# wgrosche/AIrcraft

Hardware: AMD Instinct MI355X
Metric: MPC horizon-steps/sec (6-DoF+NN-surrogate RK4, step + A,B sensitivities) at H=50, batch=4096 (higher is better)
Workload: dtype f32

## Files before the change

### aircraft_amd/build.py

```python
from __future__ import annotations

import glob
import os
import subprocess
import sys
from concurrent.futures import ThreadPoolExecutor

_HERE = os.path.dirname(os.path.abspath(__file__))
CSRC = os.path.join(_HERE, "csrc")
OBJ = os.path.join(_HERE, "csrc", "_obj")
OUT = os.path.join(_HERE, "libaircraft_hip.so")
HEADERS = glob.glob(os.path.join(CSRC, "*.hpp")) + [os.path.join(_HERE, "..", "include", "aircraft_hip.h")]
CFLAGS = ["--offload-arch=gfx950", "-O3", "-std=c++17", "-fPIC", "-fno-gpu-rdc", "-Wno-pass-failed", "-ffp-contract=on"]
UNIT_FLAGS = {
    "an_inst_sens_poly": ["-fno-slp-vectorize"],
    "nn_inst_wt2_mfma_sens_w2": ["-fno-slp-vectorize"],
    "nn_inst_wt8_mfma_sens": ["-DAC_CH=2", "-mllvm", "-slp-threshold=6", "-mllvm", "-amdgpu-mfma-vgpr-form"],
    "nn_inst_wt8_mfma_pair": ["-DAC_CH=2", "-mllvm", "-slp-threshold=6", "-mllvm", "-amdgpu-mfma-vgpr-form"],
    "nn_inst_wt8_f16_sens": ["-DAC_CH=2", "-mllvm", "-slp-threshold=6", "-mllvm", "-amdgpu-mfma-vgpr-form"],
    "nn_inst_wt8_f16_pair": ["-DAC_CH=2", "-mllvm", "-slp-threshold=6", "-mllvm", "-amdgpu-mfma-vgpr-form"],
}


def sources():
    return sorted(glob.glob(os.path.join(CSRC, "*.hip")))


def source_sha() -> str:
    import hashlib

    hh = hashlib.sha256()
    for f in sources() + sorted(HEADERS):
        hh.update(os.path.basename(f).encode())
        with open(f, "rb") as fh:
            hh.update(fh.read())
    hh.update(repr((CFLAGS, sorted(UNIT_FLAGS.items()))).encode())
    return hh.hexdigest()[:16]


def _deps(obj):
    d = obj + ".d"
    if not os.path.exists(d):
        return HEADERS
# ... 50 lines not shown
```

### aircraft_amd/csrc/ac_mlp.hpp

```cpp
#pragma once
#include "ac_dynamics.hpp"
#include "ac_mlp_plan.hpp"

namespace ac {

typedef float f32x4 __attribute__((ext_vector_type(4)));

#ifdef AC_HIDDEN_FP32
constexpr bool kBf16Hidden = false;
#else
constexpr bool kBf16Hidden = true;
#endif
constexpr int kHiddenFp32 = 0, kHiddenBf16 = 1, kHiddenF16 = 2;
constexpr int kDefaultHidden = kBf16Hidden ? kHiddenBf16 : kHiddenFp32;

__device__ __attribute__((noinline)) inline f32x4 mma_16x16x4_valu(float a, float b, f32x4 c) {
    const int lane = threadIdx.x & 63, col = lane & 15, g = lane >> 4;
#pragma unroll
    for (int k = 0; k < 4; ++k) {
        const float bk = __shfl(b, col + 16 * k, 64);
#pragma unroll
        for (int r = 0; r < 4; ++r) c[r] = fmaf(__shfl(a, 4 * g + r + 16 * k, 64), bk, c[r]);
    }
    return c;
}

template <bool USE_MFMA> AC_DI f32x4 mma_16x16x4(float a, float b, f32x4 c) {
    if constexpr (USE_MFMA) return __builtin_amdgcn_mfma_f32_16x16x4f32(a, b, c, 0, 0, 0);
    else return mma_16x16x4_valu(a, b, c);
}

AC_DI float act_tanh(float x) {
    const float e = __builtin_amdgcn_exp2f(x * 2.8853900817779268f);
    return 1.0f - 2.0f * __builtin_amdgcn_rcpf(1.0f + e);
}

// ... 11 lines not shown

template <bool ON> struct TripleHolder {
    int tri_p = 0, tri_q = 1, tri_r = 2, tri_t = 3;
    AC_DI void set_triple(int p, int q, int r) { tri_p = p; tri_q = q; tri_r = r; }
    AC_DI void set_quad(int p, int q, int r, int t) { tri_p = p; tri_q = q; tri_r = r; tri_t = t; }
    AC_DI int tri(int i) const { return i == 0 ? tri_p : i == 1 ? tri_q : i == 2 ? tri_r : tri_t; }
};
template <> struct TripleHolder<false> {
    AC_DI int tri(int) const { return 0; }
};

template <bool ON> struct BfRingState {
    int bf_front = 0;
    const char* bf_back = nullptr;
    const float* bf_next_src = nullptr;
    int bf_next_dst = 0;
};
template <> struct BfRingState<false> {};

template <int NSLAB, int WT, bool USE_MFMA, bool TANGENT = (NSLAB == 6), bool SECOND = false, int TOFF = 0, int PAIR = 0,
          int HID = kHiddenFp32>
struct MlpEngine : TripleHolder<SECOND && NSLAB <= 10>, BfRingState<HID != kHiddenFp32> {
    static constexpr bool BF = HID != kHiddenFp32;
    static constexpr bool F16 = HID == kHiddenF16;
    static constexpr int NP = F16 ? 2 : 3;
    static constexpr int NPROD = F16 ? 3 : 6;
    using TripleHolder<SECOND && NSLAB <= 10>::tri;
    static constexpr bool kNoValue = PAIR == 2;
    static constexpr int kFirstTangent = kNoValue ? 0 : 1;
    static_assert(PAIR == 0 || (TANGENT && USE_MFMA && NSLAB == 3), "wave-pair roles: three slabs each, matrix-core flavour");
    static_assert(!BF || (TANGENT && USE_MFMA && WT == 8), "bf16 hidden layers: the width-128 sensitivity engines");
    static_assert(!TANGENT || (NSLAB >= 2 && NSLAB <= 6 && TOFF + NSLAB - kFirstTangent <= 5), "tangent mode = value + a range of the 5 input tangents");
    static constexpr int kTangents = TANGENT ? NSLAB - kFirstTangent : 0;
    static_assert(!SECOND || ((NSLAB == 9 || NSLAB == 10 || NSLAB == 21) && !TANGENT), "second-order mode: 9 (bipartite), 10 (triple) or 21 (all five inputs) slabs");
    static constexpr int kFirstOrder = !SECOND ? 0 : (NSLAB == 10 ? 3 : NSLAB == 9 ? 4 : 5);
    AC_DI static constexpr int second_a(int s) {
        constexpr int K = kFirstOrder;
        if (NSLAB == 9) return s < 7 ? 1 : 2;
        if (s <= 2 * K) return s - K;
        int m = s - 2 * K - 1;
        for (int i = 1; i < K; ++i) { if (m < K - i) return i; m -= K - i; }
        return K;
    }
    AC_DI static constexpr int second_b(int s) {
        constexpr int K = kFirstOrder;
        if (NSLAB == 9) return (s & 1) ? 3 : 4;
        if (s <= 2 * K) return s - K;
// ... 23 lines not shown
    static constexpr bool kSpread = TANGENT && NSLAB * (WT / CH) * 4 >= WT * WT + 1;
    const char* dma_src;
    unsigned dma_dst;
    int dma_last;

    AC_DI MlpEngine(const MlpPlan& pl, const float* blob, char* lds_base)
        : plan(pl), gblob(blob), lds(lds_base), ring_pos(0), snext(pl.n_streamed > 1 ? 1 : 0),
          dma_src((const char*)(blob + pl.g_off[0])), dma_dst((unsigned)pl.lds_off[0]), dma_last(0) {
        lane = threadIdx.x & 63; g = lane >> 4; wave = threadIdx.x >> 6; nwaves = blockDim.x >> 6;
    }

    AC_DI int streamed_layer(int idx) const {
        int seen = 0;
        for (int l = 0; l < plan.n_layers; ++l)
            if (plan.lds_off[l] < 0) { if (seen == idx) return l; ++seen; }
        return -1;
    }

    AC_DI void load_weights() {
        for (int l = 0; l < plan.n_layers; ++l)
            if (plan.lds_off[l] >= 0) lds_dma_copy(gblob + plan.g_off[l], lds + plan.lds_off[l], plan.bytes[l], wave, nwaves, lane);
        if constexpr (BF) {
            if (!kPairRing && plan.n_streamed > 0)
                lds_dma_copy(gblob + plan.g_off[plan.first_streamed], lds + plan.bf_region[0], kBfFront, wave, nwaves, lane);
        } else if (plan.n_streamed > 0) {
            const int l = plan.first_streamed;
            lds_dma_copy(gblob + plan.g_off[l], lds + plan.ring_off[0], plan.bytes[l], wave, nwaves, lane);
        }
        asm volatile("s_waitcnt vmcnt(0)" ::: "memory");
        __syncthreads();
    }

    AC_DI void drain() { asm volatile("s_waitcnt vmcnt(0)" ::: "memory"); }

    template <int NT, int ACT = -1>
    AC_DI void epilogue_tile(int s, int nt, const f32x4 (&o)[NT], int act_flag) {
        const bool act = ACT < 0 ? act_flag != 0 : ACT != 0;
#pragma unroll
        for (int r = 0; r < 4; ++r) {
            if constexpr (kNoValue) {
                a[s][nt][r] = o[nt][r];
            } else if (s == 0 || !kDeriv) {
                a[s][nt][r] = act ? act_tanh(o[nt][r]) : o[nt][r];
            } else if (!SECOND || s <= kFirstOrder) {
                const float h = a[0][nt][r];
                a[s][nt][r] = act ? o[nt][r] * fmaf(-h, h, 1.0f) : o[nt][r];
            } else {
// ... 130 lines not shown
                const bool more = !(s == NSLAB - 1 && nc + C >= NT);
                gemm_chunk<C, KT, NT, ACT>(wf, bias4, s, nc, o[s & 1], a[s], o[(s + 1) & 1], act, wcur, bcur, more);
            }
            if (KT == WT && NT == WT) { if (s == 0) AC_MARK(st, 9); else if (s == 1) AC_MARK(st, 10); else AC_MARK(st, 11); }
            if constexpr (PAIR != 0 && KT == WT && NT == WT) {
                if (s == 1) {
                    __syncthreads();
                    if constexpr (PAIR == 1) {
#pragma unroll
                        for (int nt = 0; nt < WT; ++nt) hx[nt * 64 + lane] = f32x4{a[0][nt][0], a[0][nt][1], a[0][nt][2], a[0][nt][3]};
                    }
                }
            }
        }
#pragma unroll
        for (int nt = 0; nt < NT; ++nt) epilogue_tile<NT, ACT>(NSLAB - 1, nt, o[(NSLAB - 1) & 1], act);
    }

    typedef __bf16 bf16x8 __attribute__((ext_vector_type(8)));
    typedef unsigned u32x4 __attribute__((ext_vector_type(4)));
    static constexpr int KC = WT / 2;
    static constexpr bool kPairRing = PAIR != 0;
    static constexpr int kBfFront = (WT / 2) * KC * NP * 1024 + 1024, kBfBack = (WT / 2) * KC * NP * 1024;

    typedef float f32x2 __attribute__((ext_vector_type(2)));
    AC_DI static unsigned cvt_pk_bf16(f32x2 xy) {
        typedef __bf16 bf16x2 __attribute__((ext_vector_type(2)));
        return __builtin_bit_cast(unsigned, __builtin_convertvector(xy, bf16x2));
    }
    AC_DI static unsigned cvt_pk_bf16(float x, float y) { return cvt_pk_bf16(f32x2{x, y}); }
    typedef _Float16 f16x8 __attribute__((ext_vector_type(8)));
    template <bool H, class A, class B> struct PickFrag { typedef A type; };
    template <class A, class B> struct PickFrag<true, A, B> { typedef B type; };
    typedef typename PickFrag<F16, bf16x8, f16x8>::type frag8;
    static constexpr float kLoScale = 2048.0f, kLoInv = 1.0f / 2048.0f;
    AC_DI static unsigned cvt_pk_f16(f32x2 xy) {
        typedef _Float16 f16x2 __attribute__((ext_vector_type(2)));
        return __builtin_bit_cast(unsigned, __builtin_convertvector(xy, f16x2));
    }
    AC_DI static float sub_f16_lo(float x, unsigned u) {
        float d;
        asm volatile("v_fma_mix_f32 %0, %1, -1.0, %2 op_sel_hi:[1,0,0]" : "=v"(d) : "v"(u), "v"(x));
        return d;
    }
    AC_DI static float sub_f16_hi(float x, unsigned u) {
        float d;
// ... 2 lines not shown
    }
    AC_DI static unsigned scale_f16_lo(float r) {
        unsigned q;
        asm volatile("v_fma_mixlo_f16 %0, %1, %2, 0" : "=v"(q) : "v"(r), "s"(kLoScale));
        return q;
    }
    AC_DI static unsigned scale_f16_hi(unsigned q, float r) {
        asm volatile("v_fma_mixhi_f16 %0, %1, %2, 0" : "+v"(q) : "v"(r), "s"(kLoScale));
        return q;
    }
    AC_DI static f32x4 mfma_bf(const frag8& w, const frag8& x, f32x4 c) {
        if constexpr (F16) return __builtin_amdgcn_mfma_f32_16x16x32_f16(w, x, c, 0, 0, 0);
        else return __builtin_amdgcn_mfma_f32_16x16x32_bf16(w, x, c, 0, 0, 0);
    }
    AC_DI static float bf_sum(float hi, float lo) {
        if constexpr (F16) return fmaf(lo, kLoInv, hi);
        else return hi + lo;
    }
    AC_DI static frag8 ds_frag(unsigned lds_addr, int off) {
        frag8 v;
        asm volatile("ds_read_b128 %0, %1 offset:%2" : "=a"(v) : "v"(lds_addr), "i"(off));
        return v;
    }
    AC_DI static void wait_frags() {
        asm volatile("s_waitcnt lgkmcnt(0)" ::: "memory");
        __builtin_amdgcn_sched_barrier(0);
    }
    AC_DI void mid_layer() {
#ifdef AC_STAMPS_MID
        AC_MARK(st, 9);
        asm volatile("s_waitcnt vmcnt(0)" ::: "memory");
        AC_MARK(st, 6);
        __syncthreads();
        AC_MARK(st, 0);
#else
        asm volatile("s_waitcnt vmcnt(0)" ::: "memory");
        __syncthreads();
#endif
        if constexpr (!kPairRing) lds_dma_copy(this->bf_next_src, lds + this->bf_next_dst, kBfFront, wave, nwaves, lane);
    }

    static constexpr int NG = WT / CH;
    static constexpr int kTail = 2;
    static constexpr int kHead = (NG - kTail) * KC;
    static constexpr int NB = NG * KC;
    static constexpr int NGAP = NPROD * CH;
// ... 47 lines not shown
    static constexpr int NU = 2 * WT + 4 * KC;
    AC_DI static constexpr int unit_slab(int S, int B, int u) {
        if (u < WT) {
            const int sb = sum_blk(u / CH);
            return sb % NB == B ? (sb < NB ? S : S - 1) : -1;
        }
        if (u < 2 * WT) {
            const int t = u - WT;
            if (!kNoValue) {
                const int tb = tanh_blk(t);
                if ((S == 0 && tb == B) || (S == 1 && tb == NB + B)) return 0;
            }
            if (S >= kFirstTangent && epi_own(S, t) && epi_own_blk(t) == B) return S;
            if (S > kFirstTangent && !epi_own(S - 1, t) && epi_blk(S - 1, t) == B) return S - 1;
            return -1;
        }
        const int pb = split_blk((u - 2 * WT) / 4, (u - 2 * WT) % 4);
        if (pb < NB) return (pb == B && S + 1 < NSLAB) ? S + 1 : -1;
        return (pb == NB + B && S > 0) ? S : -1;
    }
    AC_DI static constexpr int unit_stages(int us, int u) {
        return u < WT ? 2 : u < 2 * WT ? (!kNoValue && us == 0 ? 12 : 4) : (F16 ? 3 : 6);
    }
    AC_DI static constexpr int gap_share(int S, int B) {
        if (!F16) return 1;
        int t = 0;
        for (int u = 0; u < NU; ++u) {
            const int us = unit_slab(S, B, u);
            if (us >= 0) t += unit_stages(us, u);
        }
        const int per = (t + NGAP - 1) / NGAP;
        return per < 1 ? 1 : per;
    }
    static constexpr int kSumGap = F16 ? NGAP / 2 : 4;
    AC_DI static constexpr int gap_stage(int S, int B, int J, int n) {
        const int per = gap_share(S, B);
        int j = 0;
        for (int v = WT; v < NU + WT; ++v) {
            const int u = v % NU;
            const int us = unit_slab(S, B, u);
            if (us < 0) continue;
            if (u < WT && j < kSumGap * per) j = kSumGap * per;
            for (int k = 0; k < unit_stages(us, u); ++k, ++j)
                if ((j / per < NGAP ? j / per : NGAP - 1) == J && n-- == 0) return u * 16 + k;
        }
        return -1;
    }

    struct BfRegs {
        f32x4 o[2][WT], hi[2][WT], lo[2][WT];
        u32x4 xq[WT / 2][NP];
        frag8 w[2][CH][NP];
        unsigned la0, la1;
        const f32x4* bias4;
        f32x2 sxy[2 * WT]; float tt[WT][4];
        unsigned su[2 * WT], sa[2 * WT], sb[2 * WT];
    };
    AC_DI static void bf_pin(float& v) { asm volatile("" : "+v"(v)); }
    AC_DI static void bf_pin(unsigned& v) { asm volatile("" : "+v"(v)); }

    template <int S, int B, int U, int K> AC_DI void bf_stage(BfRegs& r) {
        constexpr int us = unit_slab(S, B, U);
        constexpr bool early = S == 0 && B < kHead;
        if constexpr (U < WT) {
#pragma unroll
            for (int e = 2 * K; e < 2 * K + 2; ++e) {
                float v = bf_sum(r.hi[us & 1][U][e], r.lo[us & 1][U][e]);
                bf_pin(v);
                r.o[us & 1][U][e] = v;
// ... 60 lines not shown

    AC_DI frag8 bf_frag(const BfRegs& r, int nt, int c, int p) const {
        return ds_frag(nt < WT / 2 ? r.la0 : r.la1, (((nt % (WT / 2)) * KC + c) * NP + p) * 1024);
    }
    template <int S, int B, int J, int N> AC_DI void bf_gap_stages(BfRegs& r) {
        constexpr int e = gap_stage(S, B, J, N);
        if constexpr (e >= 0) {
            bf_stage<S, B, e / 16, e % 16>(r);
            bf_gap_stages<S, B, J, N + 1>(r);
        }
    }

    template <int S, int B, int J> AC_DI void bf_gap(BfRegs& r) {
        constexpr int nc = blk_group(B) * CH, c = blk_chunk(B), cur = B & 1, i = J % CH, m = J / CH;
        constexpr bool more = !(S + 1 == NSLAB && B + 1 == NB);
        constexpr int nb = (B + 1) % NB, nnc = blk_group(nb) * CH, nkc = blk_chunk(nb);
        constexpr int wp = F16 ? (m == 0 ? 1 : 0) : m == 0 ? 2 : (m == 1 || m == 4 || m == 5) ? 0 : 1;
        constexpr int xp = F16 ? (m == 1 ? 1 : 0) : m == 1 ? 2 : (m == 2 || m == 4) ? 1 : 0;
        const frag8 x = __builtin_bit_cast(frag8, r.xq[c][xp]);
        if constexpr (m < NPROD - 1) r.lo[S & 1][nc + i] = mfma_bf(r.w[cur][i][wp], x, r.lo[S & 1][nc + i]);
        else r.hi[S & 1][nc + i] = mfma_bf(r.w[cur][i][wp], x, r.hi[S & 1][nc + i]);
        __builtin_amdgcn_sched_barrier(0);
        if constexpr (more && J < NP * CH) r.w[cur ^ 1][J / NP][J % NP] = bf_frag(r, nnc + J / NP, nkc, J % NP);
        static_assert(F16 || gap_stage(S, B, J, 2) < 0, "at most two stages to a gap");
        bf_gap_stages<S, B, J, 0>(r);
        __builtin_amdgcn_sched_barrier(0);
        if constexpr (J + 1 < NGAP) bf_gap<S, B, J + 1>(r);
    }

    template <int S, int B> AC_DI void bf_block(BfRegs& r) {
        constexpr int nc = blk_group(B) * CH, c = blk_chunk(B);
        constexpr int nnc = blk_group((B + 1) % NB) * CH;
        __builtin_amdgcn_sched_barrier(0);
        if constexpr (S == 0 && nc < WT / 2 && nnc >= WT / 2) { mid_layer(); __builtin_amdgcn_sched_barrier(0); }
        wait_frags();
        if constexpr (c == 0) {
#pragma unroll
            for (int i = 0; i < CH; ++i) {
                r.hi[S & 1][nc + i] = (S == 0 && !kNoValue) ? r.bias4[(nc + i) * 4 + g] : f32x4{0.f, 0.f, 0.f, 0.f};
                r.lo[S & 1][nc + i] = f32x4{0.f, 0.f, 0.f, 0.f};
            }
        }
        bf_gap<S, B, 0>(r);
        if constexpr (B + 1 == NB) {
            if (S == 0) AC_MARK(st, 9); else if (S == 1) AC_MARK(st, 10); else AC_MARK(st, 11);
            if constexpr (PAIR != 0 && S == 1) {
                __syncthreads();
                if constexpr (PAIR == 1) {
#pragma unroll
                    for (int nt = 0; nt < WT; ++nt) hx[nt * 64 + lane] = f32x4{a[0][nt][0], a[0][nt][1], a[0][nt][2], a[0][nt][3]};
                }
            }
        }
    }
    template <int I> AC_DI void bf_blocks(BfRegs& r) {
        if constexpr (I < NSLAB * NB) {
            bf_block<I / NB, I % NB>(r);
            bf_blocks<I + 1>(r);
        }
    }

    AC_DI void layer_bf(const char* wfront) {
        const frag8* wf0 = reinterpret_cast<const frag8*>(wfront) + lane;
        const frag8* wf1 = reinterpret_cast<const frag8*>(this->bf_back) + lane;
        static_assert(WT % CH == 0 && (WT / 2) % CH == 0 && CH < KC, "a chunk of output tiles lies in one half");
        static_assert((WT / 2) * KC * NP * 1024 <= 65536, "a half-layer fits the ds_read immediate offset");
        BfRegs r;
        r.la0 = (unsigned)(uintptr_t)(const __attribute__((address_space(3))) char*)(const char*)wf0;
        r.la1 = (unsigned)(uintptr_t)(const __attribute__((address_space(3))) char*)(const char*)wf1;
        r.bias4 = reinterpret_cast<const f32x4*>(wfront + kBfBack);
#pragma unroll
        for (int i = 0; i < CH; ++i)
#pragma unroll
            for (int p = 0; p < NP; ++p) r.w[0][i][p] = bf_frag(r, i, 0, p);
#pragma unroll
        for (int c = 0; c < KC; ++c) {
            u32x4 q[NP];
#pragma unroll
            for (int i = 0; i < 4; ++i) split_pair(0, c, i, q);
#pragma unroll
            for (int k = 0; k < NP; ++k) r.xq[c][k] = q[k];
        }
        bf_blocks<0>(r);
        __builtin_amdgcn_sched_barrier(0);
        constexpr int L = (NSLAB - 1) & 1;
#pragma unroll
        for (int gi = 0; gi < NG; ++gi)
#pragma unroll
            for (int i = 0; i < CH; ++i)
                if (sum_blk(gi) >= NB) {
                    if constexpr (F16) {
#pragma unroll
// ... 350 lines not shown
                for (int e = 0; e < 4; ++e) p[4 * q + e] = v[e];
            }
#pragma unroll
            for (int i = 0; i < kGroup; ++i) {
                const int sl = s0 + i;
                if (sl >= NSLAB) continue;
#pragma unroll
                for (int k = 0; k < 6; ++k) {
                    const float tot = p[i * 6 + k];
                    if (sl == 0 && !kNoValue) {
                        const float pre = tot + bias[k];
                        y[k] = act ? act_tanh(pre) : pre;
                        sp[k] = act ? fmaf(-y[k], y[k], 1.0f) : 1.0f;
                    } else if constexpr (PAIR != 0) {
                        J[k][sl - kFirstTangent] = tot;
                    } else {
                        J[k][sl - 1] = sp[k] * tot;
                    }
                }
            }
        }
    }

    AC_DI const char* acquire(int l) {
        if (plan.lds_off[l] >= 0) return lds + plan.lds_off[l];
        asm volatile("s_waitcnt vmcnt(0)" ::: "memory");
        __syncthreads();
        if constexpr (BF) {
            const float* src = gblob + plan.g_off[l];
            if constexpr (kPairRing) {
                lds_dma_copy(src, lds + plan.bf_region[0], kBfFront, wave, nwaves, lane);
                asm volatile("s_waitcnt vmcnt(0)" ::: "memory");
                __syncthreads();
                lds_dma_copy(src + kBfFront / 4, lds + plan.bf_region[1], kBfBack, wave, nwaves, lane);
                this->bf_back = lds + plan.bf_region[1];
                return lds + plan.bf_region[0];
            } else {
                const int f = this->bf_front, b = f == 2 ? 0 : f + 1, nx = b == 2 ? 0 : b + 1;
                lds_dma_copy(src + kBfFront / 4, lds + plan.bf_region[b], kBfBack, wave, nwaves, lane);
                this->bf_back = lds + plan.bf_region[b];
                const int nl = plan.streamed[snext];
                snext = (snext + 1 == plan.n_streamed) ? 0 : snext + 1;
                this->bf_next_src = gblob + plan.g_off[nl];
                this->bf_next_dst = plan.bf_region[nx];
                this->bf_front = nx;
                return lds + plan.bf_region[f];
            }
        }
        const char* wl = lds + plan.ring_off[ring_pos & 1];
        const int nl = plan.streamed[snext];
        snext = (snext + 1 == plan.n_streamed) ? 0 : snext + 1;
        if constexpr (kSpread) {
            dma_src = (const char*)(gblob + __builtin_amdgcn_readfirstlane(plan.g_off[nl]));
// ... 509 lines not shown
```

### aircraft_amd/csrc/ac_mlp_model.hpp

```cpp
#pragma once
#include <algorithm>
#include <cstdio>
#include <cstring>
#include <vector>

#include "ac_bf16_pack.hpp"
#include "ac_f16_pack.hpp"
#include "ac_mlp_plan.hpp"

namespace ac {

constexpr int kLdsBudget = 160 * 1024;

struct MlpModelInfo {
    MlpPlan plan;
    MlpPlan plan_sens;
    MlpPlan plan_rev;
    MlpPlan plan_bf;
    MlpPlan plan_bf_pair;
    MlpPlan plan_f16;
    MlpPlan plan_f16_pair;
    bool has_bf;
    int f16_gate;
    bool has_rev;
    int rev_layers;
    int wt;
    int use_mfma;
    bool has_vplan;
    ValuPlan vplan;
    int vwidth;
};

struct MlpModel : MlpModelInfo {
    std::vector<float> blob;
    std::vector<float> vimage;
    std::vector<int> widths, act;
    std::vector<std::vector<float>> W, b;
};

inline void fold_linear_layers(int n_layers, const int* widths, const int* act, const float* const* W, const float* const* b,
                               MlpModel& m) {
    struct HostLayer { int nin, nout, act; std::vector<double> W, b; };
    std::vector<HostLayer> net((size_t)n_layers);
    for (int l = 0; l < n_layers; ++l) {
        HostLayer& L = net[(size_t)l];
        L.nin = widths[l]; L.nout = widths[l + 1]; L.act = act[l] ? 1 : 0;
// ... 213 lines not shown
    }

    { const int rc = plan_lds(pl, false, err, errlen); if (rc != AC_OK) return rc; }
    MlpPlan& ps = m.plan_sens = pl;
    if (n_layers > 1) {
        ps.g_off[0] = pl.g_off[0] + pl.NT[0] * pl.KT[0] * 256;
        ps.bytes[0] = pl.bytes[0] - pl.NT[0] * pl.KT[0] * 1024;
        ps.g_off[last] = pl.g_off[last] + pl.NT[last] * pl.KT[last] * 256;
        ps.bytes[last] = 1024 + wlt_bytes;
        const int rc = plan_lds(ps, false, err, errlen);
        if (rc != AC_OK) return rc;
    }
    m.plan_bf = m.plan_f16 = ps;
    if (want_bf) {
        m.plan_bf = hidden_ring_plan(ps, bf16_layer_bytes(wt), bf16_front_bytes(wt), bf_off);
        m.plan_f16 = hidden_ring_plan(ps, f16_layer_bytes(wt), f16_front_bytes(wt), f16_off);
        if (m.plan_bf.lds_total > kLdsBudget) {
            snprintf(err, errlen, "%s", "bf16 hidden-layer ring does not fit the LDS");
            return AC_ERR_UNSUPPORTED;
        }
    }
    m.plan_bf_pair = want_bf ? drop_third_region(m.plan_bf) : ps;
    m.plan_f16_pair = want_bf ? drop_third_region(m.plan_f16) : ps;
    MlpPlan& pr = m.plan_rev = ps;
    if (want_rev) {
        for (int i = 0; i < n_hid; ++i) {
            const int e = n_layers + i;
            pr.KT[e] = wt; pr.NT[e] = wt; pr.act[e] = 0;
            pr.g_off[e] = (int)rev_off[i];
            pr.bytes[e] = (int)(rev_block_floats * 4);
        }
        pr.n_layers = n_layers + n_hid;
        m.has_rev = plan_lds(pr, true, err, errlen) == AC_OK && pr.n_streamed == 2 * n_hid &&
                    pr.lds_off[0] >= 0 && pr.lds_off[last] >= 0;
    }
    m.has_bf = want_bf;
    m.rev_layers = n_layers;
    m.wt = wt;
    m.use_mfma = use_mfma ? 1 : 0;
    m.vwidth = maxh <= 32 ? 32 : 64;
    m.has_vplan = !use_mfma && n_layers >= 2 && maxh <= 64 && build_valu_image(m, m.vwidth, m.vplan, m.vimage);
    out = std::move(m);
    return AC_OK;
}

}
// ... 1 lines not shown
```

### aircraft_amd/csrc/ac_mlp_plan.hpp

```cpp
#pragma once
#include "../../include/aircraft_hip.h"

namespace ac {

struct MlpPlan {
    int n_layers;
    int KT[AC_MAX_LAYERS];
    int NT[AC_MAX_LAYERS];
    int act[AC_MAX_LAYERS];
    int g_off[AC_MAX_LAYERS];
    int bytes[AC_MAX_LAYERS];
    int lds_off[AC_MAX_LAYERS];
    int ring_off[2];
    int n_streamed;
    int first_streamed;
    int streamed[AC_MAX_LAYERS];
    int lds_total;
    int bf_region[3];
};

struct ValuPlan {
    int n_layers;
    int act_last;
    int w_off[AC_MAX_LAYERS];
    int b_off[AC_MAX_LAYERS];
    int image_floats;
};

}
```

### aircraft_amd/csrc/ac_nn_decl.hpp

```cpp
#pragma once
#include "ac_kernels_nn.hpp"
#include "ac_hess_nn.hpp"
#include "ac_mlp_valu.hpp"
#include "ac_hess_rev.hpp"
#include "ac_wgrad.hpp"

extern template __global__ void ac::k_nn_step_sens<2, true>(const ac::DevParams, const ac::MlpPlan, const float*, const float*, const float*, float, const float*, long, long, float*, float*, float*, float*);
extern template __global__ void ac::k_nn_deriv_sens<2, true>(const ac::DevParams, const ac::MlpPlan, const float*, const float*, const float*, long, long, float*, float*, float*);
extern template __global__ void ac::k_nn_fwd<2, true, 0>(const ac::DevParams, const ac::MlpPlan, const float*, const float*, const float*, float, const float*, long, long, float*, long);
extern template __global__ void ac::k_nn_fwd<2, true, 1>(const ac::DevParams, const ac::MlpPlan, const float*, const float*, const float*, float, const float*, long, long, float*, long);
extern template __global__ void ac::k_nn_fwd<2, true, 2>(const ac::DevParams, const ac::MlpPlan, const float*, const float*, const float*, float, const float*, long, long, float*, long);
extern template __global__ void ac::k_nn_rollout<2, true>(const ac::DevParams, const ac::MlpPlan, const float*, const float*, const float*, float, long, long, float*);
extern template __global__ void ac::k_nn_stage_tensors<2, true, 0>(const ac::DevParams, const ac::MlpPlan, const float*, const float*, const float*, float, const float*, long, long, float*);
extern template __global__ void ac::k_nn_step_sens_w2<2>(const ac::DevParams, const ac::MlpPlan, const float*, const float*, const float*, float, const float*, long, long, float*, float*, float*, float*);
extern template __global__ void ac::k_nn_step_sens_pair<2>(const ac::DevParams, const ac::MlpPlan, const float*, const float*, const float*, float, const float*, long, long, float*, float*, float*, float*, long);
extern template __global__ void ac::k_nn_fwd4<2, 0>(const ac::DevParams, const ac::MlpPlan, const float*, const float*, const float*, float, const float*, long, long, float*, long);
extern template __global__ void ac::k_nn_fwd4<2, 1>(const ac::DevParams, const ac::MlpPlan, const float*, const float*, const float*, float, const float*, long, long, float*, long);
extern template __global__ void ac::k_nn_fwd4<2, 2>(const ac::DevParams, const ac::MlpPlan, const float*, const float*, const float*, float, const float*, long, long, float*, long);
extern template __global__ void ac::k_nn_rollout_coop<2, true>(const ac::DevParams, const ac::MlpPlan, const float*, const float*, const float*, float, long, long, float*);
extern template __global__ void ac::k_nn_rollout_policy_coop<2, true>(const ac::DevParams, const ac::MlpPlan, const float*, const ac::Policy, const float*, float, long, long, float*, float*);
extern template __global__ void ac::k_nn_rollout_reg<2, 1>(const ac::DevParams, const ac::MlpPlan, const float*, const float*, const float*, float, long, long, float*);
extern template __global__ void ac::k_nn_rollout_policy_reg<2, 1>(const ac::DevParams, const ac::MlpPlan, const float*, const ac::Policy, const float*, float, long, long, float*, float*);
extern template __global__ void ac::k_nn_rollout_reg<2, 2>(const ac::DevParams, const ac::MlpPlan, const float*, const float*, const float*, float, long, long, float*);
extern template __global__ void ac::k_nn_rollout_policy_reg<2, 2>(const ac::DevParams, const ac::MlpPlan, const float*, const ac::Policy, const float*, float, long, long, float*, float*);
// ... 59 lines not shown
extern template __global__ void ac::k_nn_fwd<8, false, 2>(const ac::DevParams, const ac::MlpPlan, const float*, const float*, const float*, float, const float*, long, long, float*, long);
extern template __global__ void ac::k_nn_rollout<8, false>(const ac::DevParams, const ac::MlpPlan, const float*, const float*, const float*, float, long, long, float*);
extern template __global__ void ac::k_nn_step_sens_tiled8<32>(const ac::DevParams, const ac::ValuPlan, const float*, const float*, const float*, float, const float*, long, long, float*, float*, float*, float*, unsigned*);
extern template __global__ void ac::k_nn_deriv_sens_tiled8<32>(const ac::DevParams, const ac::ValuPlan, const float*, const float*, const float*, long, long, float*, float*, float*, unsigned*);
extern template __global__ void ac::k_nn_fwd_tiled<32, 0>(const ac::DevParams, const ac::ValuPlan, const float*, const float*, const float*, float, const float*, long, long, float*);
extern template __global__ void ac::k_nn_fwd_tiled<32, 1>(const ac::DevParams, const ac::ValuPlan, const float*, const float*, const float*, float, const float*, long, long, float*);
extern template __global__ void ac::k_nn_fwd_tiled<32, 2>(const ac::DevParams, const ac::ValuPlan, const float*, const float*, const float*, float, const float*, long, long, float*);
extern template __global__ void ac::k_nn_rollout_tiled<32>(const ac::DevParams, const ac::ValuPlan, const float*, const float*, const float*, float, long, long, float*);
extern template __global__ void ac::k_nn_rollout_tiled8<32>(const ac::DevParams, const ac::ValuPlan, const float*, const float*, const float*, float, long, long, float*);
extern template __global__ void ac::k_nn_rollout_policy_tiled8<32>(const ac::DevParams, const ac::ValuPlan, const float*, const ac::Policy, const float*, float, long, long, float*, float*);
extern template __global__ void ac::k_nn_step_sens_tiled8<64>(const ac::DevParams, const ac::ValuPlan, const float*, const float*, const float*, float, const float*, long, long, float*, float*, float*, float*, unsigned*);
extern template __global__ void ac::k_nn_deriv_sens_tiled8<64>(const ac::DevParams, const ac::ValuPlan, const float*, const float*, const float*, long, long, float*, float*, float*, unsigned*);
extern template __global__ void ac::k_nn_fwd_tiled<64, 0>(const ac::DevParams, const ac::ValuPlan, const float*, const float*, const float*, float, const float*, long, long, float*);
extern template __global__ void ac::k_nn_fwd_tiled<64, 1>(const ac::DevParams, const ac::ValuPlan, const float*, const float*, const float*, float, const float*, long, long, float*);
extern template __global__ void ac::k_nn_fwd_tiled<64, 2>(const ac::DevParams, const ac::ValuPlan, const float*, const float*, const float*, float, const float*, long, long, float*);
extern template __global__ void ac::k_nn_rollout_tiled<64>(const ac::DevParams, const ac::ValuPlan, const float*, const float*, const float*, float, long, long, float*);
extern template __global__ void ac::k_nn_rollout_tiled8<64>(const ac::DevParams, const ac::ValuPlan, const float*, const float*, const float*, float, long, long, float*);
extern template __global__ void ac::k_nn_rollout_policy_tiled8<64>(const ac::DevParams, const ac::ValuPlan, const float*, const ac::Policy, const float*, float, long, long, float*, float*);
extern template __global__ void ac::k_nn_stage_tensors_rev<8>(const ac::DevParams, const ac::MlpPlan, const float*, const float*, const float*, float, const float*, long, long, int, float*, float*);
extern template __global__ void ac::k_nn_stage_tensors_rev3<8, true>(const ac::DevParams, const ac::MlpPlan, const float*, const float*, const float*, float, const float*, long, long, int, float*, float*);
extern template __global__ void ac::k_nn_stage_tensors_rev3<8, false>(const ac::DevParams, const ac::MlpPlan, const float*, const float*, const float*, float, const float*, long, long, int, float*, float*);
extern template __global__ void ac::k_nn_step_sens<8, true, ac::kHiddenF16>(const ac::DevParams, const ac::MlpPlan, const float*, const float*, const float*, float, const float*, long, long, float*, float*, float*, float*);
extern template __global__ void ac::k_nn_step_sens_pair<8, ac::kHiddenF16>(const ac::DevParams, const ac::MlpPlan, const float*, const float*, const float*, float, const float*, long, long, float*, float*, float*, float*, long);
extern template __global__ void ac::k_nn_stage_jac<2, true>(const ac::DevParams, const ac::MlpPlan, const float*, const float*, const float*, float, const float*, long, long, float*);
extern template __global__ void ac::k_mlp_wgrad<2, true>(const ac::WgradPlan, const float*, const float*, const float*, long, long, float*);
extern template __global__ void ac::k_nn_stage_jac<4, true>(const ac::DevParams, const ac::MlpPlan, const float*, const float*, const float*, float, const float*, long, long, float*);
extern template __global__ void ac::k_mlp_wgrad<4, true>(const ac::WgradPlan, const float*, const float*, const float*, long, long, float*);
extern template __global__ void ac::k_nn_stage_jac<8, true>(const ac::DevParams, const ac::MlpPlan, const float*, const float*, const float*, float, const float*, long, long, float*);
extern template __global__ void ac::k_mlp_wgrad<8, true>(const ac::WgradPlan, const float*, const float*, const float*, long, long, float*);
extern template __global__ void ac::k_nn_stage_jac<2, false>(const ac::DevParams, const ac::MlpPlan, const float*, const float*, const float*, float, const float*, long, long, float*);
extern template __global__ void ac::k_mlp_wgrad<2, false>(const ac::WgradPlan, const float*, const float*, const float*, long, long, float*);
extern template __global__ void ac::k_nn_stage_jac<4, false>(const ac::DevParams, const ac::MlpPlan, const float*, const float*, const float*, float, const float*, long, long, float*);
extern template __global__ void ac::k_mlp_wgrad<4, false>(const ac::WgradPlan, const float*, const float*, const float*, long, long, float*);
extern template __global__ void ac::k_nn_stage_jac<8, false>(const ac::DevParams, const ac::MlpPlan, const float*, const float*, const float*, float, const float*, long, long, float*);
extern template __global__ void ac::k_mlp_wgrad<8, false>(const ac::WgradPlan, const float*, const float*, const float*, long, long, float*);
```

### aircraft_amd/csrc/aircraft_hip.hip

```cpp
#include <hip/hip_runtime.h>

#include <algorithm>
#include <cmath>
#include <cstdio>
#include <cstdlib>
#include <cstring>
#include <new>
#include <vector>

#include "ac_mlp_model.hpp"
#include "ac_kernels_analytic.hpp"
#include "ac_nn_decl.hpp"
#include "ac_ilqr.hpp"
#include "ac_goal.hpp"
#include "ac_ilqr_rate.hpp"
#include "ac_shoot.hpp"
#include "ac_track.hpp"
#include "ac_hess.hpp"
#include "ac_hess_adj.hpp"
#include "ac_hess_nn.hpp"
#include "ac_hess_rev.hpp"
#include "ac_select.hpp"
#include "ac_vjp.hpp"
#include "ac_trim.hpp"
// ... 35 lines not shown

int hip_fail(hipError_t e, const char* what) {
    snprintf(g_err, sizeof(g_err), "%s: %s", what, hipGetErrorString(e));
    return AC_ERR_HIP;
}
int fail(int code, const char* msg) {
    snprintf(g_err, sizeof(g_err), "%s", msg);
    return code;
}
#define AC_HIP(call)                                           \
    do {                                                       \
        hipError_t e_ = (call);                                \
        if (e_ != hipSuccess) return hip_fail(e_, #call);      \
    } while (0)

}

struct ac_handle : MlpModelInfo {
    DevParams dp;
    int device;
    int num_cus;
    bool no_pair;
    bool all_pair;
    bool has_linear, has_poly, has_mlp;
    int hidden_route;
    float* d_rev_scratch;
    size_t rev_scratch_floats;
    float* d_blob;
    size_t blob_floats;
    float* d_vblob;
    float* d_wgimg;
    WgradPlan wg;
    unsigned* d_queue;
    float* d_hess_ws;
    size_t hess_ws_floats;
    float* d_hess_ws2;
    size_t hess_ws2_floats;
    float* d_poly_tab;
    float* d_track;
    TrackDev track;
    const void* lds_fn[48];
    int lds_bytes_set[48];
    int n_lds_fn;
    int vjp_route;
    int cgrad_grid;
    char last_name[64];
// ... 315 lines not shown
    int ndev = 0;
    if (hipGetDeviceCount(&ndev) != hipSuccess || ndev == 0) {
        snprintf(g_err, sizeof(g_err), "no HIP device visible");
        return AC_ERR_NO_DEVICE;
    }
    ac_handle* h = new (std::nothrow) ac_handle();
    if (!h) return AC_ERR_BAD_ARG;
    memset(h, 0, sizeof(*h));
    h->dp.p = *params;
    {
        hipError_t e = hipGetDevice(&h->device);
        if (e != hipSuccess) { delete h; return hip_fail(e, "hipGetDevice"); }
    }
    {
        int cus = 0;
        if (hipDeviceGetAttribute(&cus, hipDeviceAttributeMultiprocessorCount, h->device) == hipSuccess) h->num_cus = cus;
    }
#ifdef AC_DIAG_ENV
    {
        const char* e = getenv("AIRCRAFT_HIP_NO_PAIR");
        h->no_pair = e && e[0] == '1';
        const char* ea = getenv("AIRCRAFT_HIP_ALL_PAIR");
        h->all_pair = ea && ea[0] == '1';
        const char* er = getenv("AIRCRAFT_HIP_HIDDEN_ROUTE");
        if (er && !strcmp(er, "bf16")) h->hidden_route = AC_HIDDEN_BF16;
        if (er && !strcmp(er, "f16")) h->hidden_route = AC_HIDDEN_F16;
    }
#endif
#if defined(AC_STAMPS) || defined(AC_CLOCKS)
    h->no_pair = true;
#endif
    {
        hipError_t e = hipMalloc(&h->d_queue, 256);
        if (e == hipSuccess) e = hipMemset(h->d_queue, 0, 256);
        if (e != hipSuccess) { if (h->d_queue) (void)hipFree(h->d_queue); delete h; return hip_fail(e, "hipMalloc(work queue)"); }
    }
    *out = h;
    return AC_OK;
}

int ac_destroy(ac_handle* h) {
    AC_ENTER(h);
    if (!h) return AC_ERR_BAD_ARG;
    if (h->d_blob) (void)hipFree(h->d_blob);
    if (h->d_vblob) (void)hipFree(h->d_vblob);
    if (h->d_wgimg) (void)hipFree(h->d_wgimg);
// ... 328 lines not shown
            const long rem = n % per_round;
            if (rem > 0 && rem <= 32 * cus) { n_main = n - rem; n_pair = rem; }
            if (h->all_pair) { n_main = 0; n_pair = n; }
        }
        const bool bf = kBf16Hidden && h->use_mfma && h->wt == 8 && h->has_bf;
        const bool f16_ok = bf && h->f16_gate == F16_GATE_OK;
        if (h->hidden_route == AC_HIDDEN_F16 && !f16_ok) return fail(AC_ERR_UNSUPPORTED, hidden_f16_refusal(h));
        const bool f16 = f16_ok && h->hidden_route != AC_HIDDEN_BF16;
        if (h->use_mfma && h->wt == 2 && h->dp.p.substeps <= 1) {
            const int lds = ((h->plan_sens.lds_total + 15) & ~15) + kSensW2AccBytes;
            if (lds <= 80 * 1024) {
                const int grid = (int)std::min<long>((n + 63) / 64, 2 * cus);
                return launch_kernel(h, st, "k_nn_step_sens_w2", k_nn_step_sens_w2<2>, grid, kBlock, lds, h->dp, h->plan_sens, h->d_blob,
                                 X, U, dt, dt_per_unit, n, blk, Xn, A, Bm, c);
            }
        }
        if (n_main > 0) {
#ifndef AC_NO_PERSIST
            const int grid = (int)std::min<long>((n_main + 63) / 64, cus);
#else
            const int grid = (int)((n_main + 63) / 64);
#endif
            const MlpPlan& plan = f16 ? h->plan_f16 : bf ? h->plan_bf : engine_plan(h);
            auto launch_main = [&](auto kern) {
                return launch_kernel(h, st, "k_nn_step_sens", kern, grid, kBlock, plan.lds_total, h->dp, plan, h->d_blob, X, U, dt,
                                 dt_per_unit, n_main, blk, Xn, A, Bm, c);
            };
            const int rc_m = f16 ? launch_main(k_nn_step_sens<8, true, kHiddenF16>)
                                 : instance(pick_wt_mfma(h, [&](auto WT, auto MF) { return launch_main(k_nn_step_sens<WT(), MF()>); }),
                                            kNoNnInstance);
            if (rc_m != AC_OK) return rc_m;
        }
        if (n_pair > 0) {
            const int grid_p = (int)((n_pair + 31) / 32);
            const MlpPlan& plan_p = f16 ? h->plan_f16_pair : bf ? h->plan_bf_pair : h->plan_sens;
            const int lds_p = plan_p.lds_total + 2 * h->wt * 1024 + 2 * 16 * 36 * (int)sizeof(float);
            auto launch_pair = [&](auto kern) {
                return launch_kernel(h, st, n_main == 0 ? "k_nn_step_sens_pair" : nullptr, kern, grid_p, kBlock, lds_p, h->dp, plan_p,
                                 h->d_blob, X, U, dt, dt_per_unit, n, blk, Xn, A, Bm, c, n_main);
            };
            return f16 ? launch_pair(k_nn_step_sens_pair<8, kHiddenF16>)
                       : instance(pick<2, 4, 8>(h->wt, [&](auto WT) { return launch_pair(k_nn_step_sens_pair<WT()>); }), kNoNnInstance);
        }
        return AC_OK;
    }
    const int upb = 16 * (h->dp.p.model_kind == AC_MODEL_POLY ? AnalyticSensN<AC_MODEL_POLY>::value : AnalyticSensN<AC_MODEL_DEFAULT>::value);
    static_assert(AnalyticSensN<AC_MODEL_DEFAULT>::value == AnalyticSensN<AC_MODEL_LINEAR>::value, "grid size below");
    const int grid_an = (int)((n + upb - 1) / upb);
    with_analytic_model(h, [&](auto M) {
        if (h->dp.p.substeps > 1) hipLaunchKernelGGL((k_step_sens<M(), true>), grid_an, kBlock, 0, st, h->dp, X, U, dt, dt_per_unit, n, blk, Xn, A, Bm, c);
        else hipLaunchKernelGGL((k_step_sens<M(), false>), grid_an, kBlock, 0, st, h->dp, X, U, dt, dt_per_unit, n, blk, Xn, A, Bm, c);
// ... 1892 lines not shown
```

Measured before the change: 138.6 million.

## Stream f16 hidden-layer weights through a double-buffered LDS ring with DMA interleaved into MFMA gaps

Adds a ring-of-two-slots mode for the f16 sensitivity kernel. Each streamed layer's full front and back weights land in one LDS slot, and the next layer's weights are prefetched by per-wave global_load_lds pieces issued inside otherwise idle MFMA gap stages. This removes the separate mid-layer back-half copy and the serialized staging it causes. The cost is extra LDS (one more region), which can lower occupancy. The old path stays available as a Ring3 instance chosen by an env var or when the plan does not fit.

After: 140.2 million (median of 6 runs). +1.1%, better.

```diff
diff --git a/aircraft_amd/build.py b/aircraft_amd/build.py
--- a/aircraft_amd/build.py
+++ b/aircraft_amd/build.py
@@ -19,6 +19,7 @@
     "nn_inst_wt8_mfma_pair": ["-DAC_CH=2", "-mllvm", "-slp-threshold=6", "-mllvm", "-amdgpu-mfma-vgpr-form"],
     "nn_inst_wt8_f16_sens": ["-DAC_CH=2", "-mllvm", "-slp-threshold=6", "-mllvm", "-amdgpu-mfma-vgpr-form"],
     "nn_inst_wt8_f16_pair": ["-DAC_CH=2", "-mllvm", "-slp-threshold=6", "-mllvm", "-amdgpu-mfma-vgpr-form"],
+    "nn_inst_wt8_f16_sens_r3": ["-DAC_CH=2", "-mllvm", "-slp-threshold=6", "-mllvm", "-amdgpu-mfma-vgpr-form"],
 }
 
 
diff --git a/aircraft_amd/csrc/ac_mlp.hpp b/aircraft_amd/csrc/ac_mlp.hpp
--- a/aircraft_amd/csrc/ac_mlp.hpp
+++ b/aircraft_amd/csrc/ac_mlp.hpp
@@ -11,7 +11,7 @@
 #else
 constexpr bool kBf16Hidden = true;
 #endif
-constexpr int kHiddenFp32 = 0, kHiddenBf16 = 1, kHiddenF16 = 2;
+constexpr int kHiddenFp32 = 0, kHiddenBf16 = 1, kHiddenF16 = 2, kHiddenF16Ring3 = 3;
 constexpr int kDefaultHidden = kBf16Hidden ? kHiddenBf16 : kHiddenFp32;
 
 __device__ __attribute__((noinline)) inline f32x4 mma_16x16x4_valu(float a, float b, f32x4 c) {
@@ -69,7 +69,8 @@
           int HID = kHiddenFp32>
 struct MlpEngine : TripleHolder<SECOND && NSLAB <= 10>, BfRingState<HID != kHiddenFp32> {
     static constexpr bool BF = HID != kHiddenFp32;
-    static constexpr bool F16 = HID == kHiddenF16;
+    static constexpr bool F16 = HID == kHiddenF16 || HID == kHiddenF16Ring3;
+    static constexpr bool kRing4 = HID == kHiddenF16 && PAIR == 0;
     static constexpr int NP = F16 ? 2 : 3;
     static constexpr int NPROD = F16 ? 3 : 6;
     using TripleHolder<SECOND && NSLAB <= 10>::tri;
@@ -139,7 +140,8 @@
             if (plan.lds_off[l] >= 0) lds_dma_copy(gblob + plan.g_off[l], lds + plan.lds_off[l], plan.bytes[l], wave, nwaves, lane);
         if constexpr (BF) {
             if (!kPairRing && plan.n_streamed > 0)
-                lds_dma_copy(gblob + plan.g_off[plan.first_streamed], lds + plan.bf_region[0], kBfFront, wave, nwaves, lane);
+                lds_dma_copy(gblob + plan.g_off[plan.first_streamed], lds + plan.bf_region[0], kRing4 ? kBfFront + kBfBack : kBfFront,
+                             wave, nwaves, lane);
         } else if (plan.n_streamed > 0) {
             const int l = plan.first_streamed;
             lds_dma_copy(gblob + plan.g_off[l], lds + plan.ring_off[0], plan.bytes[l], wave, nwaves, lane);
@@ -316,6 +318,8 @@
     static constexpr int KC = WT / 2;
     static constexpr bool kPairRing = PAIR != 0;
     static constexpr int kBfFront = (WT / 2) * KC * NP * 1024 + 1024, kBfBack = (WT / 2) * KC * NP * 1024;
+    static constexpr int kRing4Pieces = (kBfFront + kBfBack) >> 10;
+    static constexpr int kRing4PerWave = (kRing4Pieces + 3) / 4;
 
     typedef float f32x2 __attribute__((ext_vector_type(2)));
     AC_DI static unsigned cvt_pk_bf16(f32x2 xy) {
@@ -364,6 +368,7 @@
         asm volatile("ds_read_b128 %0, %1 offset:%2" : "=a"(v) : "v"(lds_addr), "i"(off));
         return v;
     }
+    AC_DI static unsigned lds_addr(const char* p) { return (unsigned)(uintptr_t)(const __attribute__((address_space(3))) char*)p; }
     AC_DI static void wait_frags() {
         asm volatile("s_waitcnt lgkmcnt(0)" ::: "memory");
         __builtin_amdgcn_sched_barrier(0);
@@ -457,14 +462,17 @@
     AC_DI static constexpr int unit_stages(int us, int u) {
         return u < WT ? 2 : u < 2 * WT ? (!kNoValue && us == 0 ? 12 : 4) : (F16 ? 3 : 6);
     }
-    AC_DI static constexpr int gap_share(int S, int B) {
-        if (!F16) return 1;
+    AC_DI static constexpr int block_stages(int S, int B) {
         int t = 0;
         for (int u = 0; u < NU; ++u) {
             const int us = unit_slab(S, B, u);
             if (us >= 0) t += unit_stages(us, u);
         }
-        const int per = (t + NGAP - 1) / NGAP;
+        return t;
+    }
+    AC_DI static constexpr int gap_share(int S, int B) {
+        if (!F16) return 1;
+        const int per = (block_stages(S, B) + NGAP - 1) / NGAP;
         return per < 1 ? 1 : per;
     }
     static constexpr int kSumGap = F16 ? NGAP / 2 : 4;
@@ -480,6 +488,36 @@
                 if ((j / per < NGAP ? j / per : NGAP - 1) == J && n-- == 0) return u * 16 + k;
         }
         return -1;
+    }
+    AC_DI static constexpr int gap_stages(int S, int B, int J) {
+        int n = 0;
+        while (gap_stage(S, B, J, n) >= 0) ++n;
+        return n;
+    }
+
+    static constexpr int kRing4Slab0 = 2, kRing4Slab1 = NSLAB - 1;
+    struct Ring4Slab { int ord[NB > 0 ? NB : 1]; };
+    AC_DI static constexpr int ring4_count(int S) {
+        constexpr int n = kRing4Slab1 - kRing4Slab0 > 0 ? kRing4Slab1 - kRing4Slab0 : 1;
+        return (S < kRing4Slab0 || S >= kRing4Slab1) ? 0 : kRing4PerWave / n + (S - kRing4Slab0 < kRing4PerWave % n ? 1 : 0);
+    }
+    AC_DI static constexpr Ring4Slab ring4_slab(int S) {
+        Ring4Slab r{};
+        int load[NB > 0 ? NB : 1] = {}, first = 0;
+        for (int s = kRing4Slab0; s < S; ++s) first += ring4_count(s);
+        for (int b = 0; b < NB; ++b) load[b] = block_stages(S, b);
+        for (int b = 0, o = first; b < NB; ++b) {
+            int rank = 0;
+            for (int c = 0; c < NB; ++c) rank += load[c] < load[b] || (load[c] == load[b] && c < b);
+            r.ord[b] = rank < ring4_count(S) ? o++ : -1;
+        }
+        return r;
+    }
+    AC_DI static constexpr int ring4_gap(int S, int B) {
+        int best = NP * CH;
+        for (int J = NP * CH + 1; J < NGAP; ++J)
+            if (gap_stages(S, B, J) <= gap_stages(S, B, best)) best = J;
+        return best;
     }
 
     struct BfRegs {
@@ -586,6 +624,10 @@
         else r.hi[S & 1][nc + i] = mfma_bf(r.w[cur][i][wp], x, r.hi[S & 1][nc + i]);
         __builtin_amdgcn_sched_barrier(0);
         if constexpr (more && J < NP * CH) r.w[cur ^ 1][J / NP][J % NP] = bf_frag(r, nnc + J / NP, nkc, J % NP);
+        if constexpr (kRing4 && S >= kRing4Slab0 && J >= NP * CH) {
+            constexpr int ord = ring4_slab(S).ord[B];
+            if constexpr (ord >= 0 && J == ring4_gap(S, B)) ring4_piece<ord>(r.la0);
+        }
         static_assert(F16 || gap_stage(S, B, J, 2) < 0, "at most two stages to a gap");
         bf_gap_stages<S, B, J, 0>(r);
         __builtin_amdgcn_sched_barrier(0);
@@ -596,7 +638,7 @@
         constexpr int nc = blk_group(B) * CH, c = blk_chunk(B);
         constexpr int nnc = blk_group((B + 1) % NB) * CH;
         __builtin_amdgcn_sched_barrier(0);
-        if constexpr (S == 0 && nc < WT / 2 && nnc >= WT / 2) { mid_layer(); __builtin_amdgcn_sched_barrier(0); }
+        if constexpr (!kRing4 && S == 0 && nc < WT / 2 && nnc >= WT / 2) { mid_layer(); __builtin_amdgcn_sched_barrier(0); }
         wait_frags();
         if constexpr (c == 0) {
 #pragma unroll
@@ -626,12 +668,12 @@
 
     AC_DI void layer_bf(const char* wfront) {
         const frag8* wf0 = reinterpret_cast<const frag8*>(wfront) + lane;
-        const frag8* wf1 = reinterpret_cast<const frag8*>(this->bf_back) + lane;
+        const frag8* wf1 = reinterpret_cast<const frag8*>(kRing4 ? wfront + kBfFront : this->bf_back) + lane;
         static_assert(WT % CH == 0 && (WT / 2) % CH == 0 && CH < KC, "a chunk of output tiles lies in one half");
         static_assert((WT / 2) * KC * NP * 1024 <= 65536, "a half-layer fits the ds_read immediate offset");
         BfRegs r;
-        r.la0 = (unsigned)(uintptr_t)(const __attribute__((address_space(3))) char*)(const char*)wf0;
-        r.la1 = (unsigned)(uintptr_t)(const __attribute__((address_space(3))) char*)(const char*)wf1;
+        r.la0 = lds_addr((const char*)wf0);
+        r.la1 = lds_addr((const char*)wf1);
         r.bias4 = reinterpret_cast<const f32x4*>(wfront + kBfBack);
 #pragma unroll
         for (int i = 0; i < CH; ++i)
@@ -1028,13 +1070,34 @@
         }
     }
 
+    template <int ORD> AC_DI void ring4_piece(unsigned la0) {
+        static_assert(ORD >= 0 && ORD < kRing4PerWave, "issue point");
+        unsigned pc = (unsigned)(4 * ORD) << 10;
+        if constexpr (4 * ORD + 4 > kRing4Pieces) pc = ((unsigned)(kRing4Pieces - 1) - (unsigned)__builtin_amdgcn_readfirstlane(wave)) << 10;
+        const char* sb = dma_src + pc;
+        asm volatile("" : "+s"(sb));
+        __builtin_amdgcn_global_load_lds((const __attribute__((address_space(1))) void*)(sb + (size_t)la0),
+                                         (__attribute__((address_space(3))) void*)(lds + dma_dst + pc), 16, 0, 0);
+    }
+
     AC_DI const char* acquire(int l) {
         if (plan.lds_off[l] >= 0) return lds + plan.lds_off[l];
         asm volatile("s_waitcnt vmcnt(0)" ::: "memory");
         __syncthreads();
         if constexpr (BF) {
             const float* src = gblob + plan.g_off[l];
-            if constexpr (kPairRing) {
+            if constexpr (kRing4) {
+                (void)src;
+                const Ring4Step step = f16_ring4_step(plan, ring_pos, snext);
+                snext = step.snext;
+                ++ring_pos;
+                const char* wl = lds + f16_ring4_slot(plan, step.read_slot);
+                const unsigned w0 = (unsigned)__builtin_amdgcn_readfirstlane(wave) << 10;
+                dma_src = (const char*)(gblob + __builtin_amdgcn_readfirstlane(plan.g_off[step.next_layer])) + w0 -
+                          (unsigned)__builtin_amdgcn_readfirstlane((int)lds_addr(wl));
+                dma_dst = (unsigned)__builtin_amdgcn_readfirstlane(f16_ring4_slot(plan, step.next_slot)) + w0;
+                return wl;
+            } else if constexpr (kPairRing) {
                 lds_dma_copy(src, lds + plan.bf_region[0], kBfFront, wave, nwaves, lane);
                 asm volatile("s_waitcnt vmcnt(0)" ::: "memory");
                 __syncthreads();
diff --git a/aircraft_amd/csrc/ac_mlp_model.hpp b/aircraft_amd/csrc/ac_mlp_model.hpp
--- a/aircraft_amd/csrc/ac_mlp_model.hpp
+++ b/aircraft_amd/csrc/ac_mlp_model.hpp
@@ -9,8 +9,6 @@
 #include "ac_mlp_plan.hpp"
 
 namespace ac {
-
-constexpr int kLdsBudget = 160 * 1024;
 
 struct MlpModelInfo {
     MlpPlan plan;
@@ -22,6 +20,7 @@
     MlpPlan plan_f16_pair;
     bool has_bf;
     int f16_gate;
+    int f16_ring4_lds;
     bool has_rev;
     int rev_layers;
     int wt;
@@ -281,6 +280,7 @@
     }
     m.plan_bf_pair = want_bf ? drop_third_region(m.plan_bf) : ps;
     m.plan_f16_pair = want_bf ? drop_third_region(m.plan_f16) : ps;
+    m.f16_ring4_lds = want_bf ? f16_ring4_lds(m.plan_f16, f16_front_bytes(wt)) : 0;
     MlpPlan& pr = m.plan_rev = ps;
     if (want_rev) {
         for (int i = 0; i < n_hid; ++i) {
diff --git a/aircraft_amd/csrc/ac_mlp_plan.hpp b/aircraft_amd/csrc/ac_mlp_plan.hpp
--- a/aircraft_amd/csrc/ac_mlp_plan.hpp
+++ b/aircraft_amd/csrc/ac_mlp_plan.hpp
@@ -19,6 +19,22 @@
     int bf_region[3];
 };
 
+constexpr int kLdsBudget = 160 * 1024;
+
+constexpr int f16_ring4_lds(const MlpPlan& p, int front_bytes) {
+    if (p.n_streamed < 1 || p.bf_region[0] < 0 || p.bf_region[2] < 0) return 0;
+    const int region = p.bf_region[1] - p.bf_region[0];
+    if (region != front_bytes || p.bf_region[2] - p.bf_region[1] != region || p.lds_total != p.bf_region[2] + region) return 0;
+    if (region % 1024 != 0 || p.bf_region[0] % 1024 != 0) return 0;
+    const int total = p.lds_total + region;
+    return total <= kLdsBudget ? total : 0;
+}
+constexpr int f16_ring4_slot(const MlpPlan& p, int k) { return k ? p.bf_region[2] : p.bf_region[0]; }
+struct Ring4Step { int read_slot, next_layer, next_slot, snext; };
+constexpr Ring4Step f16_ring4_step(const MlpPlan& p, int ring_pos, int snext) {
+    return Ring4Step{ring_pos & 1, p.streamed[snext], (ring_pos & 1) ^ 1, snext + 1 == p.n_streamed ? 0 : snext + 1};
+}
+
 struct ValuPlan {
     int n_layers;
     int act_last;
diff --git a/aircraft_amd/csrc/ac_nn_decl.hpp b/aircraft_amd/csrc/ac_nn_decl.hpp
--- a/aircraft_amd/csrc/ac_nn_decl.hpp
+++ b/aircraft_amd/csrc/ac_nn_decl.hpp
@@ -105,6 +105,7 @@
 extern template __global__ void ac::k_nn_stage_tensors_rev3<8, false>(const ac::DevParams, const ac::MlpPlan, const float*, const float*, const float*, float, const float*, long, long, int, float*, float*);
 extern template __global__ void ac::k_nn_step_sens<8, true, ac::kHiddenF16>(const ac::DevParams, const ac::MlpPlan, const float*, const float*, const float*, float, const float*, long, long, float*, float*, float*, float*);
 extern template __global__ void ac::k_nn_step_sens_pair<8, ac::kHiddenF16>(const ac::DevParams, const ac::MlpPlan, const float*, const float*, const float*, float, const float*, long, long, float*, float*, float*, float*, long);
+extern template __global__ void ac::k_nn_step_sens<8, true, ac::kHiddenF16Ring3>(const ac::DevParams, const ac::MlpPlan, const float*, const float*, const float*, float, const float*, long, long, float*, float*, float*, float*);
 extern template __global__ void ac::k_nn_stage_jac<2, true>(const ac::DevParams, const ac::MlpPlan, const float*, const float*, const float*, float, const float*, long, long, float*);
 extern template __global__ void ac::k_mlp_wgrad<2, true>(const ac::WgradPlan, const float*, const float*, const float*, long, long, float*);
 extern template __global__ void ac::k_nn_stage_jac<4, true>(const ac::DevParams, const ac::MlpPlan, const float*, const float*, const float*, float, const float*, long, long, float*);
diff --git a/aircraft_amd/csrc/aircraft_hip.hip b/aircraft_amd/csrc/aircraft_hip.hip
--- a/aircraft_amd/csrc/aircraft_hip.hip
+++ b/aircraft_amd/csrc/aircraft_hip.hip
@@ -81,6 +81,7 @@
     int num_cus;
     bool no_pair;
     bool all_pair;
+    bool f16_ring3;
     bool has_linear, has_poly, has_mlp;
     int hidden_route;
     float* d_rev_scratch;
@@ -442,6 +443,8 @@
         h->no_pair = e && e[0] == '1';
         const char* ea = getenv("AIRCRAFT_HIP_ALL_PAIR");
         h->all_pair = ea && ea[0] == '1';
+        const char* e3 = getenv("AIRCRAFT_HIP_F16_RING3");
+        h->f16_ring3 = e3 && e3[0] == '1';
         const char* er = getenv("AIRCRAFT_HIP_HIDDEN_ROUTE");
         if (er && !strcmp(er, "bf16")) h->hidden_route = AC_HIDDEN_BF16;
         if (er && !strcmp(er, "f16")) h->hidden_route = AC_HIDDEN_F16;
@@ -816,11 +819,14 @@
             const int grid = (int)((n_main + 63) / 64);
 #endif
             const MlpPlan& plan = f16 ? h->plan_f16 : bf ? h->plan_bf : engine_plan(h);
+            const bool ring4 = f16 && h->f16_ring4_lds > 0 && !h->f16_ring3;
+            const int lds_main = ring4 ? h->f16_ring4_lds : plan.lds_total;
             auto launch_main = [&](auto kern) {
-                return launch_kernel(h, st, "k_nn_step_sens", kern, grid, kBlock, plan.lds_total, h->dp, plan, h->d_blob, X, U, dt,
+                return launch_kernel(h, st, "k_nn_step_sens", kern, grid, kBlock, lds_main, h->dp, plan, h->d_blob, X, U, dt,
                                  dt_per_unit, n_main, blk, Xn, A, Bm, c);
             };
-            const int rc_m = f16 ? launch_main(k_nn_step_sens<8, true, kHiddenF16>)
+            const int rc_m = ring4 ? launch_main(k_nn_step_sens<8, true, kHiddenF16>)
+                                 : f16 ? launch_main(k_nn_step_sens<8, true, kHiddenF16Ring3>)
                                  : instance(pick_wt_mfma(h, [&](auto WT, auto MF) { return launch_main(k_nn_step_sens<WT(), MF()>); }),
                                             kNoNnInstance);
             if (rc_m != AC_OK) return rc_m;
diff --git a/aircraft_amd/csrc/nn_inst_wt8_f16_sens_r3.hip b/aircraft_amd/csrc/nn_inst_wt8_f16_sens_r3.hip
--- /dev/null
+++ b/aircraft_amd/csrc/nn_inst_wt8_f16_sens_r3.hip
@@ -0,0 +1,3 @@
+#include "ac_kernels_nn.hpp"
+
+template __global__ void ac::k_nn_step_sens<8, true, ac::kHiddenF16Ring3>(const ac::DevParams, const ac::MlpPlan, const float*, const float*, const float*, float, const float*, long, long, float*, float*, float*, float*);
```
